# infil00p/openbts-ttsou

Hardware: AMD Instinct MI355X
Metric: Mbursts/s (156.25-sym @ 4 sps) demod+detect (higher is better)
Workload: dtype f32

## Files before the change

### openbts-ttsou_amd/csrc/trxsig_corr.h

```cpp
#pragma once
#include "trxsig_dev.h"

namespace {

template <int SPS>
struct CorrGeom {
  static constexpr int NL = 36 * SPS;
  static constexpr int NC = (NL + 15) / 16;
  static constexpr int FRONT = 8 * SPS;
  static constexpr int WPAD0 = NC * 16 + 15 * SPS + 1;
  static constexpr int WPAD = ((WPAD0 + 15) / 32) * 32 + 16;
  static constexpr int H = (5 * SPS + 1 > 12) ? 5 * SPS + 1 : 12;
  static constexpr int NS = 2 * H + 1;
  static constexpr int NE = 20 * SPS;
  static constexpr int NEQ = (NE + 15) / 16;
  static constexpr int NPAIR = (NS + 2) / 2;
};
template <typename T>
__device__ __forceinline__ T &rec_slot(T *rec, int Bpad, int s, int b) { return rec[2 * ((size_t)(s >> 1) * Bpad + b) + (s & 1)]; }

template <int N>
__device__ __forceinline__ float add_row_shl(float acc, float v) {
  float r;
  if (N == 0) asm volatile("v_add_f32 %0, %1, %2" : "=v"(r) : "v"(v), "v"(acc));
  else asm volatile("v_add_f32_dpp %0, %1, %2 row_shl:%3 row_mask:0xf bank_mask:0xf bound_ctrl:1"
                    : "=v"(r) : "v"(v), "v"(acc), "n"(N));
  return r;
}
template <int SPS, int I>
__device__ __forceinline__ float energy_chain_step(float acc, const float (&nrm)[CorrGeom<SPS>::NEQ]) {
  if constexpr (I < CorrGeom<SPS>::NE) {
    acc = add_row_shl<I % 16>(acc, nrm[I / 16]);
    return energy_chain_step<SPS, I + 1>(acc, nrm);
  } else {
    return acc;
  }
}
template <int SPS, int I>
__device__ __forceinline__ float energy_chain(float acc, const float (&nrm)[CorrGeom<SPS>::NEQ]) {
  asm volatile("s_nop 1");
  return energy_chain_step<SPS, I>(acc, nrm);
}

template <int SPS>
struct CorrIn {
  typedef CorrGeom<SPS> G;
  static constexpr int NW = (CorrGeom<SPS>::NL + 15) / 16;
  cx w[NW];
  cx e[CorrGeom<SPS>::NEQ];
  int b;
  bool live, good;
  __device__ __forceinline__ void stage_window(cx *W, int r) const {
#pragma unroll
    for (int i = 0; i < NW; i++) {
      const int q = r + 16 * i;
      if (q < G::NL) W[G::FRONT + q] = w[i];
    }
  }
  __device__ __forceinline__ void stage_norms(float *ef, int r) const {
#pragma unroll
    for (int q = 0; q < G::NEQ; q++) {
      const int i = r + 16 * q;
      if (i < G::NE) ef[i] = norm2(e[q]);
    }
  }
};

template <int SPS>
__device__ __forceinline__ void corr_issue(CorrIn<SPS> &in, int b, int B, int r, const cx *__restrict__ samples,
                                           const int32_t *__restrict__ offset, const int32_t *__restrict__ length) {
  typedef CorrGeom<SPS> G;
  in.b = b;
  in.live = b < B;
  int off = 0, len = 0;
  if (in.live) { off = offset[b]; len = length[b]; }
  in.good = in.live && (off >= 0) && (len >= 92 * SPS) && (len <= 157 * SPS) && (len % SPS == 0);
  const cx *x = samples + (in.good ? off : 0);
#pragma unroll
  for (int i = 0; i < CorrIn<SPS>::NW; i++) {
    const int q = r + 16 * i;
    in.w[i] = (in.good && q < G::NL) ? x[56 * SPS + q] : mk(0, 0);
  }
#pragma unroll
  for (int q = 0; q < G::NEQ; q++) {
    const int i = r + 16 * q;
    in.e[q] = (in.good && i < G::NE) ? x[i] : mk(0, 0);
  }
}

template <int SPS, bool REC, bool EFIRST = false, unsigned TAPCLS = TRX_TAPS_GENERIC, typename IN = CorrIn<SPS>>
__device__ __forceinline__ void corr_round(const IN &in, cx *W, float4 *E, int lane, int r, const cx (&tap)[16],
                                           cx *__restrict__ rec, int Bpad, int &M_out, float &energy_out) {
  typedef CorrGeom<SPS> G;
  auto stage_norms = [&] { in.stage_norms(reinterpret_cast<float *>(E), r); };
  auto sum_norms = [&] {
    float energy = 0.0f;
#pragma unroll
    for (int i4 = 0; i4 < (G::NE + 3) / 4; i4++) {
      const float4 e = E[i4];
      energy = energy + e.x;
      if (4 * i4 + 1 < G::NE) energy = energy + e.y;
      if (4 * i4 + 2 < G::NE) energy = energy + e.z;
      if (4 * i4 + 3 < G::NE) energy = energy + e.w;
    }
    return energy;
  };
  float energy = 0.0f;
  if (EFIRST) {
    stage_norms();
    wave_lds_fence();
    energy = sum_norms();
    asm volatile("" : "+v"(energy));
    wave_lds_fence();
  }
  for (int q = r; q < G::FRONT; q += 16) W[q] = mk(0, 0);
  for (int q = G::FRONT + G::NL + r; q < G::WPAD; q += 16) W[q] = mk(0, 0);
  in.stage_window(W, r);
  if (!EFIRST) stage_norms();
  wave_lds_fence();
  if (!EFIRST) energy = sum_norms();

  float bestP = 0.0f;
  int bestT = -1;
  cx cval[G::NC];
  constexpr int CG = (SPS == 4) ? TRX_CORR_CG : 1;
  constexpr int UPC = 16 / SPS;
  constexpr int NU = UPC * (CG - 1) + 16;
#pragma unroll
  for (int c0 = 0; c0 < G::NC; c0 += CG) {
    cx sv[NU];
#pragma unroll
    for (int u = 0; u < NU; u++) sv[u] = W[r + 16 * c0 + SPS * u];
#pragma unroll
    for (int cc = 0; cc < CG; cc++) {
      if (c0 + cc < G::NC) {
        cx acc = mk(0, 0);
#pragma unroll
        for (int k = 15; k >= 0; k--) acc = cadd(acc, cmul_tap(sv[UPC * cc + k], tap[k], (TAPCLS >> (2 * k)) & 3));
        cval[c0 + cc] = acc;
      }
    }
  }
  wave_lds_fence();
#pragma unroll
  for (int c = 0; c < G::NC; c++) {
    const int t = r + 16 * c;
    if (t < G::NL) {
      W[t] = cval[c];
      const float p = norm2(cval[c]);
      if (p > bestP) { bestP = p; bestT = t; }
    }
  }
#pragma unroll
  for (int m = 1; m < 16; m <<= 1) {
    const float oP = __shfl_xor(bestP, m, 64);
    const int oT = __shfl_xor(bestT, m, 64);
    const bool take = (oP > bestP) || (oP == bestP && oT >= 0 && (bestT < 0 || oT < bestT));
    if (take) { bestP = oP; bestT = oT; }
  }
  wave_lds_fence();

  M_out = bestT;
  energy_out = energy;
  if (REC && in.live) {
    const int M = bestT;
    auto slot = [&](int s) {
      cx v = mk(0, 0);
      if (s < G::NS) {
        const int lag = M - G::H + s;
        if (lag >= 0 && lag < G::NL) v = W[lag];
      } else if (s == G::NS) {
        v = mk(__int_as_float(in.good ? M : -2), energy);
      }
      return v;
    };
    for (int j = r; j < G::NPAIR; j += 16) {
      const cx a = slot(2 * j), c = slot(2 * j + 1);
      reinterpret_cast<float4 *>(rec)[(size_t)j * Bpad + in.b] = make_float4(a.r, a.i, c.r, c.i);
    }
  }
  wave_lds_fence();
  (void)lane;
}


inline unsigned tap_classes(const TrxTables *hT, int tsc) {
  unsigned m = 0;
  for (int k = 0; k < 16; k++) {
    const trx_c32 a = hT->mid_ctap[tsc][k];
    const unsigned c = (a.r == 1.0f || a.r == -1.0f) ? 1u : ((a.i == 1.0f || a.i == -1.0f) ? 2u : 0u);
    m |= c << (2 * k);
  }
  return m;
}

}
```

### openbts-ttsou_amd/csrc/trxsig_dev.h

```cpp
#pragma once
#include <hip/hip_runtime.h>
#include <hip/hip_fp16.h>
#include <stdint.h>

#include <type_traits>

#include "trxsig_tables.h"
#include "trxsig_launch.h"

#ifndef TRX_CORR_CG
#define TRX_CORR_CG 3
#endif
#ifndef TRX_CORR_WPS
#define TRX_CORR_WPS 1
#endif
#ifndef TRX_CORR_ROUNDS
#define TRX_CORR_ROUNDS 1
#endif
#ifndef TRX_DEMOD_WAVES
#define TRX_DEMOD_WAVES 4
#endif

namespace {

typedef trx_c32 cx;

__device__ __forceinline__ cx mk(float r, float i) { cx z; z.r = r; z.i = i; return z; }
__device__ __forceinline__ cx cmul(cx x, cx a) { return mk(x.r * a.r - x.i * a.i, x.r * a.i + x.i * a.r); }
__device__ __forceinline__ cx cmul_sum(cx x, cx a, float nai) { return mk(x.r * a.r + x.i * nai, x.r * a.i + x.i * a.r); }
__device__ __forceinline__ float neg_opaque(float v) {
  float r = -v;
  asm volatile("" : "+v"(r));
  return r;
}
__device__ __forceinline__ cx cmul_sum(cx x, cx a) { return cmul_sum(x, a, neg_opaque(a.i)); }
__device__ __forceinline__ cx cmulr(cx x, float a) { return mk(x.r * a, x.i * a); }
__device__ __forceinline__ cx cadd(cx x, cx a) { return mk(x.r + a.r, x.i + a.i); }
__device__ __forceinline__ float norm2(cx x) { return x.i * x.i + x.r * x.r; }
__device__ __forceinline__ cx cinv(cx x) { float n = norm2(x); return mk(x.r / n, -x.i / n); }
__device__ __forceinline__ cx cdiv(cx x, cx a) { return cmul(x, cinv(a)); }

template <int CTRL>
__device__ __forceinline__ float dpp_f(float v) {
  return __int_as_float(__builtin_amdgcn_update_dpp(0, __float_as_int(v), CTRL, 0xf, 0xf, true));
}
template <int CTRL>
__device__ __forceinline__ int dpp_i(int v) { return __builtin_amdgcn_update_dpp(0, v, CTRL, 0xf, 0xf, true); }
__device__ __forceinline__ float wave_sum_any_order(float v) {
  v += dpp_f<0xB1>(v);
  v += dpp_f<0x4E>(v);
  v += dpp_f<0x141>(v);
  v += dpp_f<0x140>(v);
  const float r0 = __int_as_float(__builtin_amdgcn_readlane(__float_as_int(v), 0));
  const float r1 = __int_as_float(__builtin_amdgcn_readlane(__float_as_int(v), 16));
  const float r2 = __int_as_float(__builtin_amdgcn_readlane(__float_as_int(v), 32));
  const float r3 = __int_as_float(__builtin_amdgcn_readlane(__float_as_int(v), 48));
  return ((r0 + r1) + r2) + r3;
}
__device__ __forceinline__ void argmax_take(float &P, int &T, float oP, int oT) {
  const bool take = (oP > P) || (oP == P && oT >= 0 && (T < 0 || oT < T));
  P = take ? oP : P;
  T = take ? oT : T;
}
__device__ __forceinline__ void wave_argmax(float &P, int &T) {
  argmax_take(P, T, dpp_f<0xB1>(P), dpp_i<0xB1>(T));
  argmax_take(P, T, dpp_f<0x4E>(P), dpp_i<0x4E>(T));
  argmax_take(P, T, dpp_f<0x141>(P), dpp_i<0x141>(T));
  argmax_take(P, T, dpp_f<0x140>(P), dpp_i<0x140>(T));
  float bp = __int_as_float(__builtin_amdgcn_readlane(__float_as_int(P), 0));
  int bt = __builtin_amdgcn_readlane(T, 0);
#pragma unroll
  for (int r = 16; r < 64; r += 16)
    argmax_take(bp, bt, __int_as_float(__builtin_amdgcn_readlane(__float_as_int(P), r)), __builtin_amdgcn_readlane(T, r));
  P = bp; T = bt;
}

typedef float v2f __attribute__((ext_vector_type(2)));
__device__ __forceinline__ v2f pk(cx z) { v2f v = {z.r, z.i}; return v; }
__device__ __forceinline__ v2f pk_cmul(v2f x, v2f a) {
  v2f p, q, r;
  asm("v_pk_mul_f32 %0, %1, %2 op_sel_hi:[0,1]" : "=v"(p) : "v"(x), "v"(a));
  asm("v_pk_mul_f32 %0, %1, %2 op_sel:[1,1] op_sel_hi:[1,0]" : "=v"(q) : "v"(x), "v"(a));
  asm("v_pk_add_f32 %0, %1, %2 neg_lo:[0,1]" : "=v"(r) : "v"(p), "v"(q));
  return r;
}
__device__ __forceinline__ v2f pk_mul(v2f x, v2f a) {
  v2f r;
  asm("v_pk_mul_f32 %0, %1, %2" : "=v"(r) : "v"(x), "v"(a));
  return r;
}
template <int HI>
__device__ __forceinline__ v2f pk_mul_tap(v2f x, v2f t) {
  v2f r;
  if (HI) asm("v_pk_mul_f32 %0, %1, %2 op_sel:[0,1] op_sel_hi:[1,1]" : "=v"(r) : "v"(x), "v"(t));
  else asm("v_pk_mul_f32 %0, %1, %2 op_sel_hi:[1,0]" : "=v"(r) : "v"(x), "v"(t));
  return r;
}
__device__ __forceinline__ v2f pk_csub(v2f x, v2f a) {
  v2f r;
  asm("v_pk_add_f32 %0, %1, %2 neg_lo:[0,1] neg_hi:[0,1]" : "=v"(r) : "v"(x), "v"(a));
  return r;
}
__device__ __forceinline__ cx unpk(v2f v) { return mk(v.x, v.y); }
__device__ __forceinline__ v2f pk_cadd(v2f x, v2f a) {
  v2f r;
  asm("v_pk_add_f32 %0, %1, %2" : "=v"(r) : "v"(x), "v"(a));
  return r;
}

struct SmpC32 {
  static constexpr int kBytes = 8;
  static __device__ __forceinline__ cx ld(const void *base, long long i) { return reinterpret_cast<const cx *>(base)[i]; }
  typedef cx raw_t;
  static __device__ __forceinline__ raw_t ldraw(const void *base, long long i) { return reinterpret_cast<const cx *>(base)[i]; }
  static __device__ __forceinline__ raw_t zero() { return mk(0, 0); }
  static __device__ __forceinline__ cx widen(raw_t r) { return r; }
  static __device__ __forceinline__ float4 ld2(const void *base, long long first, int q) {
    return reinterpret_cast<const float4 *>(reinterpret_cast<const cx *>(base) + first)[q];
  }
};
struct SmpF16 {
  static constexpr int kBytes = 4;
  static __device__ __forceinline__ cx ld(const void *base, long long i) {
    const float2 v = __half22float2(reinterpret_cast<const __half2 *>(base)[i]);
    return mk(v.x, v.y);
  }
  typedef unsigned raw_t;
  static __device__ __forceinline__ raw_t ldraw(const void *base, long long i) { return reinterpret_cast<const unsigned *>(base)[i]; }
  static __device__ __forceinline__ raw_t zero() { return 0u; }
  static __device__ __forceinline__ cx widen(raw_t r) {
    const float2 v = __half22float2(*reinterpret_cast<const __half2 *>(&r));
    return mk(v.x, v.y);
  }
  static __device__ __forceinline__ float4 ld2(const void *base, long long first, int q) {
    const uint2 u = reinterpret_cast<const uint2 *>(reinterpret_cast<const __half2 *>(base) + first)[q];
    const float2 a = __half22float2(*reinterpret_cast<const __half2 *>(&u.x)), b = __half22float2(*reinterpret_cast<const __half2 *>(&u.y));
    return make_float4(a.x, a.y, b.x, b.y);
  }
};

struct TapArg { float v[32]; };

#define TRX_TAPS_GENERIC 0u
template <int SPS> struct TapPattern {
  static constexpr unsigned value = (SPS == 4) ? 0x19999999u : 0x99999999u;
};
__device__ __forceinline__ float fma_steer(float a, float b, float c) {
  float r;
  asm("v_fma_f32 %0, %1, %2, %3 ; steering" : "=v"(r) : "v"(a), "v"(b), "v"(c));
  return r;
}
__device__ __forceinline__ float fma_steer_s(float a, float b_sgpr, float c) {
  float r;
  asm("v_fma_f32 %0, %1, %2, %3 ; steering" : "=v"(r) : "v"(a), "s"(b_sgpr), "v"(c));
  return r;
}
__device__ __forceinline__ cx cmul_tap(cx x, cx a, int cls) {
  if (cls == 1) {
    const float p = x.i * a.i, q = x.r * a.i;
    cx z;
    asm("v_fma_f32 %0, %2, %4, -%5 ; exact-product\n\tv_fma_f32 %1, %3, %4, %6 ; exact-product"
        : "=&v"(z.r), "=v"(z.i) : "v"(x.r), "v"(x.i), "s"(a.r), "v"(p), "v"(q));
    return z;
  }
  if (cls == 2) {
    const float p = x.r * a.r, q = x.i * a.r;
    cx z;
    asm("v_fma_f32 %0, %3, -%4, %5 ; exact-product\n\tv_fma_f32 %1, %2, %4, %6 ; exact-product"
        : "=&v"(z.r), "=v"(z.i) : "v"(x.r), "v"(x.i), "s"(a.i), "v"(p), "v"(q));
    return z;
  }
  return cmul(x, a);
}

#define TRX_PI_F 3.14159274101257324f
#define TRX_2PI_F 6.28318548202514648f

template <int N>
__device__ __forceinline__ float row_shl(float v) {
  if (N == 0) return v;
  return __int_as_float(__builtin_amdgcn_update_dpp(0, __float_as_int(v), 0x100 + N, 0xf, 0xf, true));
}

__device__ __forceinline__ void lds_barrier() {
  asm volatile("s_waitcnt lgkmcnt(0)\n\ts_barrier" ::: "memory");
}
__device__ __forceinline__ void wave_lds_fence() {
  __builtin_amdgcn_fence(__ATOMIC_RELEASE, "wavefront");
  __builtin_amdgcn_wave_barrier();
  __builtin_amdgcn_fence(__ATOMIC_ACQUIRE, "wavefront");
}

__device__ __forceinline__ float dev_range_reduce(float arg) {
  if (arg > 1.0F) arg = arg - (ceilf(arg) - 1.0F);
  if (arg < 0.0F) arg = arg + ceilf(-arg);
  return arg;
}
__device__ __forceinline__ float dev_sin_lookup(const float *__restrict__ sinT, float x) {
  const float arg = dev_range_reduce(x * (1 / TRX_2PI_F));
  const float argT = arg * (float)TRX_TABLESIZE;
  int argI = (int)argT;
  argI = argI < 0 ? 0 : (argI > TRX_TABLESIZE ? TRX_TABLESIZE : argI);
  const float delta = argT - argI;
  const float iDelta = 1.0F - delta;
  return iDelta * sinT[argI] + delta * sinT[argI + 1];
}
#define TRX_FSHIFT_MAXPHASE 25000.0f
__device__ __forceinline__ cx dev_expj_lookup(const TrxTables *__restrict__ T, float x) {
  const float arg = dev_range_reduce(x * (1 / TRX_2PI_F));
  const float argT = arg * (float)TRX_TABLESIZE;
  int argI = (int)argT;
  argI = argI < 0 ? 0 : (argI > TRX_TABLESIZE ? TRX_TABLESIZE : argI);
  const float delta = argT - argI;
  const float iDelta = 1.0F - delta;
  return mk(iDelta * T->cosT[argI] + delta * T->cosT[argI + 1], iDelta * T->sinT[argI] + delta * T->sinT[argI + 1]);
}
__device__ __forceinline__ float dev_sinc(const float *__restrict__ sinT, float x) {
  if ((x >= 0.01F) || (x <= -0.01F)) return dev_sin_lookup(sinT, x) / x;
  return 1.0F;
}

}
```

### openbts-ttsou_amd/csrc/trxsig_normal.hip

```cpp
#include "trxsig_bisect.h"
#include "trxsig_corr.h"
#include "trxsig_demod.h"
#include "trxsig_rxgen.h"

#ifndef TRX_RXC_WPS
#define TRX_RXC_WPS 1
#endif
#ifndef TRX_RXD_WPS
#define TRX_RXD_WPS 1
#endif

namespace {

template <int SPS, unsigned TAPCLS>
__global__ __launch_bounds__(256, TRX_CORR_WPS) void k_tsc_corr(const TrxTables *__restrict__ T,
                                                  const cx *__restrict__ samples,
                                                  const int32_t *__restrict__ offset,
                                                  const int32_t *__restrict__ length, int B, TapArg taps,
                                                  cx *__restrict__ rec, int Bpad) {
  typedef CorrGeom<SPS> G;
  static_assert(8 * G::WPAD >= 4 * G::NE, "the energy norms are staged in the row itself");
  __shared__ __attribute__((aligned(16))) cx rows[16][G::WPAD];
  (void)T;
  const int lane = threadIdx.x & 63, wave = threadIdx.x >> 6;
  const int row = lane >> 4, r = lane & 15;
  const int slot = wave * 4 + row;

  cx tap[16];
#pragma unroll
  for (int k = 0; k < 16; k++) tap[k] = mk(taps.v[2 * k], taps.v[2 * k + 1]);

  typedef CorrIn<SPS> In;
  In in[TRX_CORR_ROUNDS];
#pragma unroll
  for (int i = 0; i < TRX_CORR_ROUNDS; i++)
    corr_issue<SPS>(in[i], (blockIdx.x * TRX_CORR_ROUNDS + i) * 16 + slot, B, r, samples, offset, length);
#pragma unroll
  for (int i = 0; i < TRX_CORR_ROUNDS; i++) {
    int M;
    float energy;
    corr_round<SPS, true, true, TAPCLS, In>(in[i], rows[slot], reinterpret_cast<float4 *>(rows[slot]), lane, r, tap, rec, Bpad, M, energy);
  }
}


#ifdef TRX_TUNING_BUILD
template <int SPS>
__global__ __launch_bounds__(64) void k_tsc_peak(const TrxTables *__restrict__ T,
                                                 const cx *__restrict__ rec, int Bpad, int B, int tsc,
                                                 float detect_thresh, float energy_thresh,
                                                 uint8_t *__restrict__ flags, cx *__restrict__ amp_out,
                                                 float *__restrict__ toa_out,
                                                 float *__restrict__ avgpwr_out) {
  typedef CorrGeom<SPS> G;
  __shared__ cx loc[26][64];
  __shared__ float pw[G::NS][64];
  const int lane = threadIdx.x;
  const int b = blockIdx.x * 64 + lane;
  const bool live = b < B;
  const int bb = live ? b : B - 1;

  const cx meta = rec_slot(rec, Bpad, G::NS, bb);
  const int M = __float_as_int(meta.r);
  const float energy = meta.i;
  const bool good = M != -2;
#pragma unroll
  for (int s = 0; s < G::NS; s++) {
    const cx v = rec_slot(rec, Bpad, s, bb);
    pw[s][lane] = norm2(v);
    const int j = s - (G::H - 12);
    if (j >= 0 && j < 24) {
      const int lag = M - 12 + j;
      loc[j][lane] = (lag > G::NL - 2) ? mk(0, 0) : v;
    }
  }
  loc[24][lane] = mk(0, 0);
  loc[25][lane] = mk(0, 0);

  float peakIx;
  const cx peak = peak_bisect<64>(T->sinc_grid, loc, lane, M, &peakIx);

  float toa = peakIx;
  cx amp = peak;
  bool detected = false;
  const bool energy_ok = good && (energy_thresh < 0.0f ||
                                  energy / (float)(unsigned)G::NE > energy_thresh * energy_thresh);
  if (!(toa < 0.0f) && !(toa > (float)G::NL) && good) {
    const int p = (int)rintf(toa);
    float valley = 0.0f;
    int numRms = 0;
#pragma unroll
    for (int i = 2 * SPS; i <= 5 * SPS; i++) {
      const int lo = p - i, hi = p + i;
      int slo = lo - M + G::H, shi = hi - M + G::H;
      slo = slo < 0 ? 0 : slo; shi = shi > G::NS - 1 ? G::NS - 1 : shi;
      const float vlo = pw[slo][lane], vhi = pw[shi][lane];
      if (lo >= 0) { valley += vlo; numRms++; }
      if (hi < G::NL) { valley += vhi; numRms++; }
    }
    if (numRms < 2) {
      amp = mk(0, 0);
    } else {
      const float RMS = (float)((double)sqrtf(valley / (float)numRms) + 0.00001);
      const float peakToMean = sqrtf(norm2(amp)) / RMS;
      amp = cdiv(amp, T->mid_gain[tsc]);
      toa = toa - T->mid_toa[tsc];
      toa = toa - (float)((66 - 56) * SPS);
      detected = peakToMean > detect_thresh;
    }
  } else {
    amp = mk(0, 0);
  }
  if (!energy_ok) { amp = mk(0, 0); toa = 0.0f; detected = false; }

  if (live) {
    uint8_t fl = 0;
    if (!good) fl = TRXSIG_F_BADLEN;
    else fl = (energy_ok ? TRXSIG_F_ENERGY : 0) | (detected ? TRXSIG_F_DETECT : 0);
    flags[b] = fl;
    amp_out[b] = amp;
    toa_out[b] = toa;
    if (avgpwr_out) avgpwr_out[b] = good ? energy / (float)(unsigned)G::NE : 0.0f;
  }
}


template <int SPS>
struct Peak8Geom {
  typedef CorrGeom<SPS> G;
  static constexpr int NV = 2 * (3 * SPS + 1);
  static constexpr int O_PW = 26 * 2;
  static constexpr int O_V = O_PW + ((G::NS + 3) & ~3);
  static constexpr int STRIDE = O_V + ((NV + 3) & ~3);
};

template <int SPS>
__global__ __launch_bounds__(256, 8) void k_tsc_peak8(const TrxTables *__restrict__ T, const cx *__restrict__ rec, int Bpad,
                                                   int B, cx gain_inv, float mid_toa, float detect_thresh,
                                                   float energy_thresh, uint8_t *__restrict__ flags,
                                                   cx *__restrict__ amp_out, float *__restrict__ toa_out,
                                                   float *__restrict__ avgpwr_out) {
  typedef CorrGeom<SPS> G;
  typedef Peak8Geom<SPS> P8;
  __shared__ __attribute__((aligned(16))) float stab[32][24];
  __shared__ __attribute__((aligned(16))) float scratch[32][P8::STRIDE];
  {
    float tv[3];
#pragma unroll
    for (int k = 0; k < 3; k++) { const int ix = threadIdx.x * 3 + k; tv[k] = T->sinc_grid[16 * (ix / 24)][ix % 24]; }
#pragma unroll
    for (int k = 0; k < 3; k++) { const int ix = threadIdx.x * 3 + k; stab[ix / 24][ix % 24] = tv[k]; }
  }
  const int lane = threadIdx.x & 63;
  const int r = lane & 7;
  const int slot = threadIdx.x >> 3;
  const int b = blockIdx.x * 32 + slot;
  const bool live = b < B;
  const int bb = live ? b : B - 1;
  float *S = scratch[slot];
  cx *loc = reinterpret_cast<cx *>(S);
  float *pw = S + P8::O_PW, *V = S + P8::O_V;

  const cx meta = rec_slot(rec, Bpad, G::NS, bb);
  const int M = __float_as_int(meta.r);
  const float energy = meta.i;
  const bool good = M != -2;
#pragma unroll
  for (int s0 = 0; s0 < G::NS; s0 += 8) {
    const int sl = s0 + r;
    if (sl < G::NS) {
      const cx v = rec_slot(rec, Bpad, sl, bb);
      pw[sl] = norm2(v);
      const int j = sl - (G::H - 12);
      if (j >= 0 && j < 24) loc[j] = (M - 12 + j > G::NL - 2) ? mk(0, 0) : v;
    }
  }
  if (r < 2) loc[24 + r] = mk(0, 0);
  __syncthreads();

  int e = 0;
  asm volatile("" : "+v"(e));
  bool active = true;
  cx peak = mk(0, 0);
  {
    const int rel2 = kFusedRel2.v[r], rel1 = kFusedRel1.v[r];
#pragma unroll
    for (int st = 0; st < 4; st++) {
      const int inc_last = 128 >> (2 * st);
      const int el = e + (rel2 >> 2) * inc_last;
      float srow[24];
      if (st < 3) {
        const float4 *rw = reinterpret_cast<const float4 *>(stab[(el & 511) >> 4]);
#pragma unroll
        for (int q = 0; q < 6; q++) {
          const float4 t4 = rw[q];
          srow[4 * q] = t4.x; srow[4 * q + 1] = t4.y; srow[4 * q + 2] = t4.z; srow[4 * q + 3] = t4.w;
        }
      } else {
        fused_row(T, el, srow);
      }
      const cx pt = fused_point(loc, el, rel2 & 3, srow);
      fused_decide<8, 2, false>(pt, lane, 2 * inc_last, e, active, peak);
    }
    {
      float srow[24];
      fused_row(T, e, srow);
      const cx pt = fused_point(loc, e, rel1 & 3, srow);
      fused_decide<8, 1, false>(pt, lane, 1, e, active, peak);
    }
    float srow[24];
    fused_row(T, e, srow);
    peak = fused_point(loc, e, 1, srow);
    asm volatile("" : "+v"(peak.r), "+v"(peak.i));
  }
  cx amp;
  float toa;
  bool detected, energy_ok;
  fused_tail<SPS, 8>([&](int lag) { const int sl = lag - M + G::H; return (sl < 0 || sl >= G::NS) ? 0.0f : pw[sl]; }, V, r, M, e,
                     peak, good, energy, gain_inv, mid_toa, detect_thresh, energy_thresh, amp, toa, detected, energy_ok);
  if (live && r == 0) {
    uint8_t fl = 0;
    if (!good) fl = TRXSIG_F_BADLEN;
    else fl = (energy_ok ? TRXSIG_F_ENERGY : 0) | (detected ? TRXSIG_F_DETECT : 0);
    flags[b] = fl;
    amp_out[b] = amp;
    toa_out[b] = toa;
    if (avgpwr_out) avgpwr_out[b] = good ? energy / (float)(unsigned)G::NE : 0.0f;
  }
}



#endif

#ifndef TRX_PEAK2_THREADS
#define TRX_PEAK2_THREADS 512
#endif
constexpr int kPeak2Threads = TRX_PEAK2_THREADS;
template <int SPS>
__global__ __launch_bounds__(kPeak2Threads) void k_tsc_peak2(const TrxTables *__restrict__ T, const cx *__restrict__ rec, int Bpad,
                                                   int B, cx gain_inv, float mid_toa, float detect_thresh,
                                                   float energy_thresh, uint8_t *__restrict__ flags,
                                                   cx *__restrict__ amp_out, float *__restrict__ toa_out,
                                                   float *__restrict__ avgpwr_out) {
  typedef CorrGeom<SPS> G;
  constexpr int NL = G::NL, NE = G::NE, NP = 3 * SPS + 3;
  __shared__ __attribute__((aligned(16))) SincLds stab;
  const int tid = threadIdx.x;
  const int h = tid & 1;
  const int b = blockIdx.x * (kPeak2Threads / 2) + (tid >> 1);
  const bool live = b < B;
  const int bb = live ? b : B - 1;
#ifdef TRX_PEAK_PROBE
  long long pt_[16] = {0};
  int pk_ = 0;
#define TRX_STAMP() pt_[pk_++] = clock64()
#else
#define TRX_STAMP()
#endif
  TRX_STAMP();

  float4 tv[3072 / kPeak2Threads];
  sinc_lds_issue<kPeak2Threads>(T, tid, tv);
  const cx meta = rec_slot(rec, Bpad, G::NS, bb);
  const int M = __float_as_int(meta.r);
  const float energy = meta.i;
  const bool good = M != -2;
  const float4 *rec4 = reinterpret_cast<const float4 *>(rec);
  cx q[23];
  {
    constexpr int S0 = G::H - 12, P0 = S0 >> 1;
    float4 pw[12];
#pragma unroll
    for (int i = 0; i < 12; i++) pw[i] = rec4[(size_t)(P0 + h + i) * Bpad + bb];
#pragma unroll
    for (int k = 0; k < 23; k++) {
      const int ix = k + 2 * h;
      const float4 p4 = pw[((S0 + k) >> 1) - P0];
      const cx v = ((S0 + k) & 1) ? mk(p4.z, p4.w) : mk(p4.x, p4.y);
      q[k] = (M - 12 + ix > NL - 2) ? mk(0, 0) : v;
    }
  }
  cx vmine_[NP];
  constexpr int VLO = G::H - (5 * SPS + 1), VHI = G::H + (2 * SPS - 1);
  if constexpr ((VLO & 1) == 0 && (VHI & 1) == 0) {
    float4 pv[(NP + 1) / 2];
#pragma unroll
    for (int i = 0; i < (NP + 1) / 2; i++) pv[i] = rec4[(size_t)(((h ? VHI : VLO) >> 1) + i) * Bpad + bb];
#pragma unroll
    for (int k = 0; k < NP; k++) vmine_[k] = (k & 1) ? mk(pv[k >> 1].z, pv[k >> 1].w) : mk(pv[k >> 1].x, pv[k >> 1].y);
  } else {
#pragma unroll
    for (int k = 0; k < NP; k++) vmine_[k] = rec_slot(rec, Bpad, (h ? VHI : VLO) + k, bb);
  }
  sinc_lds_store<kPeak2Threads>(stab, tid, tv);
  TRX_STAMP();
  __syncthreads();
  TRX_STAMP();

  int e;
  const cx peak = pair_bisect(stab, q, h, e);
  TRX_STAMP();
  const float early = (float)(M - 1) + (float)e * 0.001953125f;
  float toa = early + 1.0f;
  cx amp = peak;
  bool detected = false;
  const bool energy_ok = good && (energy_thresh < 0.0f || energy / (float)(unsigned)NE > energy_thresh * energy_thresh);
  const bool sane = !(toa < 0.0f) && !(toa > (float)NL) && good;
  if (sane) {
    const int pk = (int)rintf(toa);
    const int a = pk - M + 1;
    float plo[NP], phi[NP];
#pragma unroll
    for (int k = 0; k < NP; k++) {
      const float mine = norm2(vmine_[k]);
      const float other = __int_as_float(__builtin_amdgcn_update_dpp(0, __float_as_int(mine), 0xB1, 0xf, 0xf, true));
      plo[k] = h ? other : mine; phi[k] = h ? mine : other;
    }
    float valley = 0.0f;
#pragma unroll
    for (int i = 2 * SPS; i <= 5 * SPS; i++) {
      const int t = 5 * SPS - i, u = i - 2 * SPS;
      const float vlo = a == 0 ? plo[t] : (a == 1 ? plo[t + 1] : plo[t + 2]);
      const float vhi = a == 0 ? phi[u] : (a == 1 ? phi[u + 1] : phi[u + 2]);
      valley = valley + vlo;
      valley = valley + vhi;
    }
    int nlo = (pk < 5 * SPS ? pk : 5 * SPS) - 2 * SPS + 1;
    int nhi = (NL - 1 - pk < 5 * SPS ? NL - 1 - pk : 5 * SPS) - 2 * SPS + 1;
    nlo = nlo < 0 ? 0 : nlo; nhi = nhi < 0 ? 0 : nhi;
    const int numRms = nlo + nhi;
    if (numRms < 2) {
      amp = mk(0, 0);
    } else {
      const float RMS = (float)((double)sqrtf(valley / (float)numRms) + 0.00001);
      const float peakToMean = sqrtf(norm2(amp)) / RMS;
      amp = cmul(amp, gain_inv);
      toa = toa - mid_toa;
      toa = toa - (float)((66 - 56) * SPS);
      detected = peakToMean > detect_thresh;
    }
  } else {
    amp = mk(0, 0);
  }
  if (!energy_ok) { amp = mk(0, 0); toa = 0.0f; detected = false; }

  if (live && h == 0) {
    uint8_t fl = 0;
    if (!good) fl = TRXSIG_F_BADLEN;
    else fl = (energy_ok ? TRXSIG_F_ENERGY : 0) | (detected ? TRXSIG_F_DETECT : 0);
    flags[b] = fl;
    amp_out[b] = amp;
    toa_out[b] = toa;
    if (avgpwr_out) avgpwr_out[b] = good ? energy / (float)(unsigned)G::NE : 0.0f;
  }
#ifdef TRX_PEAK_PROBE
  TRX_STAMP();
  if (live && avgpwr_out) {
    long long v = 0;
    for (int k = 1; k < 16; k++) if ((b & 15) == k) v = pt_[k] - pt_[0];
    if (h == 0) avgpwr_out[b] = (float)v;
  }
#endif
#undef TRX_STAMP
}

template <int SPS, unsigned TAPCLS>
__global__ __launch_bounds__(256, TRX_RXC_WPS) void k_tsc_corr_rx(TrxRxGen a, int B, TapArg taps, cx *__restrict__ rec, int Bpad) {
  static_assert(SPS == 4, "the fused front end is the 260 : 96 resampler");
  typedef CorrGeom<SPS> G;
  constexpr int XCAP = 160;
  static_assert(G::WPAD >= XCAP, "the raw stretch is parked in the burst's own row");
  __shared__ __attribute__((aligned(16))) cx rows[16][G::WPAD];
  __shared__ float4 tpb_s[RXG_NT];
  if (threadIdx.x < RXG_NT) tpb_s[threadIdx.x] = a.tpb[threadIdx.x];
  __syncthreads();
  const int lane = threadIdx.x & 63, wave = threadIdx.x >> 6;
  const int row = lane >> 4, r = lane & 15;
  const int slot = wave * 4 + row;
  cx tap[16];
#pragma unroll
  for (int k = 0; k < 16; k++) tap[k] = mk(taps.v[2 * k], taps.v[2 * k + 1]);
  const int b = blockIdx.x * 16 + slot;
  CorrIn<SPS> in;
  in.b = b; in.live = b < B; in.good = in.live;
  const RxBurst u = rx_burst(a, in.live ? b : 0);
  const int jlo = rx_index(u.g0, a.skipD).j0 - 3;
  cx *X = rows[slot];
  {
    short2 v[XCAP / 16];
#pragma unroll
    for (int i = 0; i < XCAP / 16; i++) v[i] = rx_raw(a, u.s, jlo + r + 16 * i);
#pragma unroll
    for (int i = 0; i < XCAP / 16; i++) X[r + 16 * i] = rx_widen(a, v[i]);
  }
  wave_lds_fence();
  {
    static_assert(G::NL % 16 == 0 && G::NE % 16 == 0, "every lane owns a sample in every round");
    const int nb = rx_boundary(u.g0);
    RxIdx ix = rx_index(u.g0 + 56 * SPS + r, a.skipD);
#pragma unroll
    for (int i = 0; i < CorrIn<SPS>::NW; i++) {
      in.w[i] = rx_sample(X, tpb_s, jlo, ix, nb - (56 * SPS + r + 16 * i), a.w0, a.w1);
      ix = rx_step<16>(ix);
      if (i % 3 == 2) asm volatile("" : "+v"(in.w[i].r), "+v"(in.w[i].i), "+v"(in.w[i - 1].r), "+v"(in.w[i - 1].i), "+v"(in.w[i - 2].r), "+v"(in.w[i - 2].i) : : "memory");
    }
    ix = rx_index(u.g0 + r, a.skipD);
#pragma unroll
    for (int q = 0; q < G::NEQ; q++) {
      in.e[q] = rx_sample(X, tpb_s, jlo, ix, nb - (r + 16 * q), a.w0, a.w1);
      ix = rx_step<16>(ix);
      if (q % 3 == 2) asm volatile("" : "+v"(in.e[q].r), "+v"(in.e[q].i), "+v"(in.e[q - 1].r), "+v"(in.e[q - 1].i), "+v"(in.e[q - 2].r), "+v"(in.e[q - 2].i) : : "memory");
    }
  }
  wave_lds_fence();
  int M;
  float energy;
  corr_round<SPS, true, true, TAPCLS>(in, rows[slot], reinterpret_cast<float4 *>(rows[slot]), lane, r, tap, rec, Bpad, M, energy);
}

template <int SPS, bool TOL = false>
__global__ __launch_bounds__(64 * TRX_DEMOD_WAVES, TRX_RXD_WPS) void k_demod_rx(const TrxTables *__restrict__ T, TrxRxGen a, int B,
                                                                  const cx *__restrict__ amp_in, const float *__restrict__ toa_in,
                                                                  const uint8_t *__restrict__ flags, int need_mask,
                                                                  float *__restrict__ soft, uint8_t *__restrict__ hard, int nsoft,
                                                                  int stride) {
  static_assert(SPS == 4, "the fused front end is the 260 : 96 resampler");
  typedef DemodGeom<SPS, 148> G;
  constexpr int XCAP = 256;
  static_assert(G::U >= XCAP, "the raw stretch is parked in the burst's staging area");
  __shared__ cx ph[TRX_DEMOD_WAVES][G::U];
  __shared__ float4 tpb_s[RXG_NT];
  if (threadIdx.x < RXG_NT) tpb_s[threadIdx.x] = a.tpb[threadIdx.x];
  __syncthreads();
  const int lane = threadIdx.x & 63;
  const int wave = __builtin_amdgcn_readfirstlane(threadIdx.x >> 6);
  const int b = blockIdx.x * TRX_DEMOD_WAVES + wave;
  if (b >= B) return;
  float *sb = soft + (size_t)b * stride;
  uint8_t *hb = hard ? hard + (size_t)b * stride : nullptr;
  const cx amp = amp_in[b];
  const float toa = toa_in[b];
  bool enabled = fabsf(toa) <= 4096.0f;
  if (flags) enabled = enabled && (need_mask ? ((flags[b] & need_mask) == need_mask) : (flags[b] != 0));
  if (!enabled) {
    for (int m = lane; m < nsoft; m += 64) { sb[m] = 0.0f; if (hb) hb[m] = 0; }
    return;
  }
  const RxBurst u = rx_burst(a, b);
  const int jlo = rx_index(u.g0, a.skipD).j0 - 3;
  cx *X = ph[wave];
  {
    short2 v[XCAP / 64];
#pragma unroll
    for (int i = 0; i < XCAP / 64; i++) v[i] = rx_raw(a, u.s, jlo + lane + 64 * i);
#pragma unroll
    for (int i = 0; i < XCAP / 64; i++) X[lane + 64 * i] = rx_widen(a, v[i]);
  }
  wave_lds_fence();
  constexpr int NSL = (157 * SPS + 63) / 64;
  cx sv[NSL];
  {
    const int nb = rx_boundary(u.g0);
    RxIdx ix = rx_index(u.g0 + lane, a.skipD);
#pragma unroll
    for (int i = 0; i < NSL; i++) {
      sv[i] = rx_sample(X, tpb_s, jlo, ix, nb - (lane + 64 * i), a.w0, a.w1);
      ix = rx_step<64>(ix);
      if (i % 2 == 1) asm volatile("" : "+v"(sv[i].r), "+v"(sv[i].i), "+v"(sv[i - 1].r), "+v"(sv[i - 1].i) : : "memory");
    }
  }
  const int N = u.N;
  auto stage = [&](cx *P, cx inv, int lo) {
    typedef DemodGeom<SPS, 148> D;
    const int u0 = lane + lo;
    if (u0 >= 0) {
      cx *p0 = P + (u0 % SPS) * D::QLEN + u0 / SPS;
#pragma unroll
      for (int i = 0; i < NSL; i++)
        if (lane + 64 * i < N && u0 + 64 * i < D::U) p0[i * (64 / SPS)] = cmul(sv[i], inv);
    } else {
#pragma unroll
      for (int i = 0; i < NSL; i++) {
        const int uu = u0 + 64 * i;
        if (lane + 64 * i < N && uu >= 0 && uu < D::U) P[(uu % SPS) * D::QLEN + uu / SPS] = cmul(sv[i], inv);
      }
    }
  };
  if (TOL) {
    float xm = 0.0f;
#pragma unroll
    for (int i = 0; i < NSL; i++)
      if (lane + 64 * i < N) xm = max3_abs(sv[i].r, sv[i].i, xm);
    auto stage_raw = [&](cx *P, int lo) {
      typedef DemodGeom<SPS, 148> D;
      const int u0 = lane + lo;
      if (u0 >= 0) {
        cx *p0 = P + (u0 % SPS) * D::QLEN + u0 / SPS;
#pragma unroll
        for (int i = 0; i < NSL; i++)
          if (lane + 64 * i < N && u0 + 64 * i < D::U) p0[i * (64 / SPS)] = sv[i];
      } else {
#pragma unroll
        for (int i = 0; i < NSL; i++) {
          const int uu = u0 + 64 * i;
          if (lane + 64 * i < N && uu >= 0 && uu < D::U) P[(uu % SPS) * D::QLEN + uu / SPS] = sv[i];
        }
      }
    };
    if (fused_demod_tol_ex<SPS>(T, ph[wave], N, amp, toa, lane, sb, hb, nsoft, xm, stage_raw)) return;
  }
  fused_demod_ex<SPS, 64>(T, ph[wave], N, amp, toa, lane, sb, hb, nsoft, stage, [] {}, nullptr, nullptr);
}

}

int trx_rec_slots(int sps) {
  switch (sps) {
    case 1: return 2 * CorrGeom<1>::NPAIR;
    case 2: return 2 * CorrGeom<2>::NPAIR;
    case 4: return 2 * CorrGeom<4>::NPAIR;
  }
  return 0;
}

template <int S>
static void launch_tsc_detect(hipStream_t st, const TrxTables *dT, const TrxTables *hT, const trx_c32 *samples, const int32_t *off,
                              const int32_t *len, int B, int tsc, float detect_thresh, float energy_thresh,
                              trx_c32 *rec, int Bpad, uint8_t *flags, trx_c32 *amp, float *toa, float *avgpwr,
                              int variant, TrxProfiler *prof) {
  TapArg ta;
  for (int k = 0; k < 16; k++) { ta.v[2 * k] = hT->mid_ctap[tsc][k].r; ta.v[2 * k + 1] = hT->mid_ctap[tsc][k].i; }
  if (prof) prof->begin(TRXSIG_K_TSC_CORR, st);
  const dim3 cgrid((B + 16 * TRX_CORR_ROUNDS - 1) / (16 * TRX_CORR_ROUNDS));
  if (!(variant & 1) && tap_classes(hT, tsc) == TapPattern<S>::value)
    k_tsc_corr<S, TapPattern<S>::value><<<cgrid, dim3(256), 0, st>>>(dT, samples, off, len, B, ta, rec, Bpad);
  else
    k_tsc_corr<S, TRX_TAPS_GENERIC><<<cgrid, dim3(256), 0, st>>>(dT, samples, off, len, B, ta, rec, Bpad);
  if (prof) { prof->end(TRXSIG_K_TSC_CORR, st); prof->begin(TRXSIG_K_TSC_PEAK, st); }
  const trx_c32 g = hT->mid_gain[tsc];
  const float n = g.i * g.i + g.r * g.r;
  trx_c32 ginv; ginv.r = g.r / n; ginv.i = -g.i / n;
#ifdef TRX_TUNING_BUILD
  if (variant & 4) {
    k_tsc_peak<S><<<dim3((B + 63) / 64), dim3(64), 0, st>>>(dT, rec, Bpad, B, tsc, detect_thresh, energy_thresh,
                                                            flags, amp, toa, avgpwr);
  } else if (variant & 2) {
    k_tsc_peak8<S><<<dim3((B + 31) / 32), dim3(256), 0, st>>>(dT, rec, Bpad, B, ginv, hT->mid_toa[tsc], detect_thresh,
                                                              energy_thresh, flags, amp, toa, avgpwr);
  } else
#endif
  {
    k_tsc_peak2<S><<<dim3((B + kPeak2Threads / 2 - 1) / (kPeak2Threads / 2)), dim3(kPeak2Threads), 0, st>>>(dT, rec, Bpad, B, ginv, hT->mid_toa[tsc], detect_thresh,
                                                                energy_thresh, flags, amp, toa, avgpwr);
  }
  if (prof) prof->end(TRXSIG_K_TSC_PEAK, st);
}

namespace {
__global__ __launch_bounds__(256) void k_copy_verdict(const uint8_t *__restrict__ f, const cx *__restrict__ a, const float *__restrict__ t, int B,
                                                      uint8_t *__restrict__ fo, cx *__restrict__ ao, float *__restrict__ to) {
  const int b = blockIdx.x * 256 + threadIdx.x;
  if (b >= B) return;
  fo[b] = f[b]; ao[b] = a[b]; to[b] = t[b];
}
}
hipError_t trx_launch_copy_verdict(hipStream_t st, const uint8_t *flags, const trx_c32 *amp, const float *toa, int B, uint8_t *flags_out,
                                   trx_c32 *amp_out, float *toa_out) {
  if (B <= 0) return hipSuccess;
  k_copy_verdict<<<dim3((B + 255) / 256), dim3(256), 0, st>>>(flags, amp, toa, B, flags_out, amp_out, toa_out);
  return hipGetLastError();
}

hipError_t trx_launch_tsc_detect(hipStream_t st, int sps, const TrxTables *dT, const TrxTables *hT, const trx_c32 *samples,
                                 const int32_t *off, const int32_t *len, int B, int tsc,
                                 float detect_thresh, float energy_thresh, trx_c32 *rec, int Bpad,
                                 uint8_t *flags, trx_c32 *amp, float *toa, float *avgpwr, int variant,
                                 TrxProfiler *prof) {
  if (B <= 0) return hipSuccess;
  switch (sps) {
    case 1: launch_tsc_detect<1>(st, dT, hT, samples, off, len, B, tsc, detect_thresh, energy_thresh, rec, Bpad, flags, amp, toa, avgpwr, variant, prof); break;
    case 2: launch_tsc_detect<2>(st, dT, hT, samples, off, len, B, tsc, detect_thresh, energy_thresh, rec, Bpad, flags, amp, toa, avgpwr, variant, prof); break;
    case 4: launch_tsc_detect<4>(st, dT, hT, samples, off, len, B, tsc, detect_thresh, energy_thresh, rec, Bpad, flags, amp, toa, avgpwr, variant, prof); break;
    default: return hipErrorInvalidValue;
  }
  return hipGetLastError();
}

hipError_t trx_launch_rx_normal(hipStream_t st, const TrxTables *dT, const TrxTables *hT, const TrxRxGen &gen, int B, int tsc,
                                float detect_thresh, float energy_thresh, trx_c32 *rec, int Bpad, uint8_t *flags, trx_c32 *amp,
                                float *toa, float *avgpwr, float *soft, uint8_t *hard, int nsoft, int stride, int generic_taps,
                                TrxProfiler *prof, int soft_tolerance) {
  if (B <= 0) return hipSuccess;
  if (nsoft > 148 || gen.nb <= 0) return hipErrorInvalidValue;
  constexpr int S = 4;
  TapArg ta;
  for (int k = 0; k < 16; k++) { ta.v[2 * k] = hT->mid_ctap[tsc][k].r; ta.v[2 * k + 1] = hT->mid_ctap[tsc][k].i; }
  if (prof) prof->begin(TRXSIG_K_TSC_CORR, st);
  const dim3 cgrid((B + 15) / 16);
  if (!generic_taps && tap_classes(hT, tsc) == TapPattern<S>::value)
    k_tsc_corr_rx<S, TapPattern<S>::value><<<cgrid, dim3(256), 0, st>>>(gen, B, ta, rec, Bpad);
  else
    k_tsc_corr_rx<S, TRX_TAPS_GENERIC><<<cgrid, dim3(256), 0, st>>>(gen, B, ta, rec, Bpad);
  if (prof) { prof->end(TRXSIG_K_TSC_CORR, st); prof->begin(TRXSIG_K_TSC_PEAK, st); }
  const trx_c32 g = hT->mid_gain[tsc];
  const float n = g.i * g.i + g.r * g.r;
  trx_c32 ginv; ginv.r = g.r / n; ginv.i = -g.i / n;
  k_tsc_peak2<S><<<dim3((B + kPeak2Threads / 2 - 1) / (kPeak2Threads / 2)), dim3(kPeak2Threads), 0, st>>>(dT, rec, Bpad, B, ginv, hT->mid_toa[tsc], detect_thresh, energy_thresh,
                                                              flags, amp, toa, avgpwr);
  if (prof) prof->end(TRXSIG_K_TSC_PEAK, st);
  if (nsoft > 0) {
    if (prof) prof->begin(TRXSIG_K_DEMOD, st);
    if (soft_tolerance)
      k_demod_rx<S, true><<<dim3((B + TRX_DEMOD_WAVES - 1) / TRX_DEMOD_WAVES), dim3(64 * TRX_DEMOD_WAVES), 0, st>>>(
          dT, gen, B, amp, toa, flags, TRXSIG_F_DETECT, soft, hard, nsoft, stride);
    else
      k_demod_rx<S><<<dim3((B + TRX_DEMOD_WAVES - 1) / TRX_DEMOD_WAVES), dim3(64 * TRX_DEMOD_WAVES), 0, st>>>(
          dT, gen, B, amp, toa, flags, TRXSIG_F_DETECT, soft, hard, nsoft, stride);
    if (prof) prof->end(TRXSIG_K_DEMOD, st);
  }
  return hipGetLastError();
}

hipError_t trx_launch_rx_demod(hipStream_t st, const TrxTables *dT, const TrxRxGen &gen, int B, const trx_c32 *amp, const float *toa,
                               const uint8_t *flags, int need_mask, float *soft, uint8_t *hard, int nsoft, int stride, TrxProfiler *prof,
                               int soft_tolerance) {
  if (B <= 0 || nsoft <= 0) return hipSuccess;
  if (nsoft > 148 || gen.nb <= 0) return hipErrorInvalidValue;
  if (prof) prof->begin(TRXSIG_K_DEMOD, st);
  if (soft_tolerance)
    k_demod_rx<4, true><<<dim3((B + TRX_DEMOD_WAVES - 1) / TRX_DEMOD_WAVES), dim3(64 * TRX_DEMOD_WAVES), 0, st>>>(dT, gen, B, amp, toa, flags,
                                                                                                                  need_mask, soft, hard, nsoft, stride);
  else
    k_demod_rx<4><<<dim3((B + TRX_DEMOD_WAVES - 1) / TRX_DEMOD_WAVES), dim3(64 * TRX_DEMOD_WAVES), 0, st>>>(dT, gen, B, amp, toa, flags, need_mask,
                                                                                                            soft, hard, nsoft, stride);
  if (prof) prof->end(TRXSIG_K_DEMOD, st);
  return hipGetLastError();
}

hipError_t trx_launch_demod(hipStream_t st, int sps, const TrxTables *dT, const trx_c32 *samples,
                            const int32_t *off, const int32_t *len, int B, const trx_c32 *amp,
                            const float *toa, const uint8_t *flags, int need_mask, float *soft,
                            uint8_t *hard, int nsoft, int stride, TrxProfiler *prof, int soft_tolerance) {
  if (B <= 0) return hipSuccess;
  const dim3 grid((B + TRX_DEMOD_WAVES - 1) / TRX_DEMOD_WAVES), block(64 * TRX_DEMOD_WAVES);
  if (prof) prof->begin(TRXSIG_K_DEMOD, st);
#define TRX_DEMOD_CASE(S)                                                                                          \
  case S:                                                                                                          \
    if (nsoft <= 148 && soft_tolerance)                                                                            \
      k_demod<S, false, 148, SmpC32, true><<<grid, block, 0, st>>>(dT, samples, off, len, B, amp, toa, flags, need_mask, soft, hard, \
                                                     nsoft, stride);                                              \
    else if (nsoft <= 148)                                                                                         \
      k_demod<S, false, 148><<<grid, block, 0, st>>>(dT, samples, off, len, B, amp, toa, flags, need_mask, soft, hard, \
                                                     nsoft, stride);                                              \
    else                                                                                                           \
      k_demod<S, false, 157><<<grid, block, 0, st>>>(dT, samples, off, len, B, amp, toa, flags, need_mask, soft, hard, \
                                                     nsoft, stride);                                              \
    break;
  switch (sps) {
    TRX_DEMOD_CASE(1)
    TRX_DEMOD_CASE(2)
    TRX_DEMOD_CASE(4)
    default: return hipErrorInvalidValue;
  }
#undef TRX_DEMOD_CASE
  if (prof) prof->end(TRXSIG_K_DEMOD, st);
  return hipGetLastError();
}
```

Measured before the change: 629.5.

## Specialize correlator for near-unit taps with runtime magnitude screen and pad skipping

Correlation kernels are now templated on a 64-bit tap spec that records which taps are exactly ±1 or ±j (tiny imaginary part) and their signs. For those taps the complex multiply becomes a plain add or subtract. Tap products that only touch zero padding are skipped at compile time. A wave-wide screen on the window's exponent range (finite values, bounded dynamic range) decides at runtime whether the trimmed path is numerically safe. Otherwise the full path runs, with a NaN/Inf poison fix-up so the output still matches generic semantics. This adds code size, five kernel instantiations, and extra DPP reductions per round.

```diff
diff --git a/openbts-ttsou_amd/csrc/trxsig_corr.h b/openbts-ttsou_amd/csrc/trxsig_corr.h
--- a/openbts-ttsou_amd/csrc/trxsig_corr.h
+++ b/openbts-ttsou_amd/csrc/trxsig_corr.h
@@ -1,4 +1,6 @@
 #pragma once
+#include <cmath>
+
 #include "trxsig_dev.h"
 
 namespace {
@@ -57,6 +59,22 @@
       if (q < G::NL) W[G::FRONT + q] = w[i];
     }
   }
+  __device__ __forceinline__ void window_extremes(unsigned &lo, unsigned &hi) const {
+    static_assert(G::NL % 16 == 0, "every lane holds NW samples of the window");
+    lo = 0xffffffffu; hi = 0u;
+#pragma unroll
+    for (int i = 0; i < NW; i++) {
+      const unsigned a = __float_as_uint(w[i].r) & 0x7fffffffu, c = __float_as_uint(w[i].i) & 0x7fffffffu;
+      lo = min(lo, min(a, c));
+      hi = max(hi, max(a, c));
+    }
+  }
+  __device__ __forceinline__ unsigned window_max() const {
+    unsigned hi = 0u;
+#pragma unroll
+    for (int i = 0; i < NW; i++) hi = max(hi, max(__float_as_uint(w[i].r) & 0x7fffffffu, __float_as_uint(w[i].i) & 0x7fffffffu));
+    return hi;
+  }
   __device__ __forceinline__ void stage_norms(float *ef, int r) const {
 #pragma unroll
     for (int q = 0; q < G::NEQ; q++) {
@@ -88,7 +106,81 @@
   }
 }
 
-template <int SPS, bool REC, bool EFIRST = false, unsigned TAPCLS = TRX_TAPS_GENERIC, typename IN = CorrIn<SPS>>
+template <int SPS>
+constexpr bool corr_pad_only(int c, int k) {
+  const int first = 16 * c + SPS * k, last = first + 15;
+  return last < CorrGeom<SPS>::FRONT || first >= CorrGeom<SPS>::FRONT + CorrGeom<SPS>::NL;
+}
+
+template <int SPS>
+__device__ __forceinline__ bool corr_screen(const CorrIn<SPS> &in, unsigned &hi) {
+  unsigned lo;
+  in.window_extremes(lo, hi);
+  lo = min(lo, (unsigned)dpp_i<0xB1>((int)lo));  hi = max(hi, (unsigned)dpp_i<0xB1>((int)hi));
+  lo = min(lo, (unsigned)dpp_i<0x4E>((int)lo));  hi = max(hi, (unsigned)dpp_i<0x4E>((int)hi));
+  lo = min(lo, (unsigned)dpp_i<0x141>((int)lo)); hi = max(hi, (unsigned)dpp_i<0x141>((int)hi));
+  lo = min(lo, (unsigned)dpp_i<0x140>((int)lo)); hi = max(hi, (unsigned)dpp_i<0x140>((int)hi));
+  const bool ok = hi < 0x7f800000u && lo >= (27u << 23) && lo + (20u << 23) >= hi;
+  return __builtin_amdgcn_ballot_w64(!ok) == 0;
+}
+
+template <int SPS>
+__device__ __forceinline__ unsigned corr_row_max(const CorrIn<SPS> &in) {
+  unsigned hi = in.window_max();
+  hi = max(hi, (unsigned)dpp_i<0xB1>((int)hi));
+  hi = max(hi, (unsigned)dpp_i<0x4E>((int)hi));
+  hi = max(hi, (unsigned)dpp_i<0x141>((int)hi));
+  return max(hi, (unsigned)dpp_i<0x140>((int)hi));
+}
+
+template <int SPS>
+__device__ __forceinline__ void corr_poison(unsigned hi, const cx *W, int r, cx (&cval)[CorrGeom<SPS>::NC]) {
+  if constexpr (SPS > 1) {
+    if (hi >= 0x7f800000u) {
+#pragma unroll
+      for (int c = 0; c < CorrGeom<SPS>::NC; c++) {
+        unsigned worst = 0u;
+#pragma unroll 1
+        for (int m = 1; m < 16 * SPS; m++) {
+          if (m % SPS == 0) continue;
+          const cx x = W[r + 16 * c + m];
+          worst = max(worst, max(__float_as_uint(x.r) & 0x7fffffffu, __float_as_uint(x.i) & 0x7fffffffu));
+        }
+        if (worst >= 0x7f800000u) cval[c] = mk(__uint_as_float(0x7fc00000u), __uint_as_float(0x7fc00000u));
+      }
+    }
+  }
+}
+
+template <int SPS, tapspec_t TAPS, bool TRIM>
+__device__ __forceinline__ void corr_sums(const cx *W, int r, const cx (&tap)[16], cx (&cval)[CorrGeom<SPS>::NC]) {
+  typedef CorrGeom<SPS> G;
+  constexpr bool SPEC = TAPS != TRX_TAPS_GENERIC;
+  constexpr int CG = (SPS == 4) ? TRX_CORR_CG : 1;
+  constexpr int UPC = 16 / SPS;
+  constexpr int NU = UPC * (CG - 1) + 16;
+#pragma unroll
+  for (int c0 = 0; c0 < G::NC; c0 += CG) {
+    cx sv[NU];
+#pragma unroll
+    for (int u = 0; u < NU; u++) sv[u] = W[r + 16 * c0 + SPS * u];
+#pragma unroll
+    for (int cc = 0; cc < CG; cc++) {
+      if (c0 + cc < G::NC) {
+        cx acc = mk(0, 0);
+#pragma unroll
+        for (int k = 15; k >= 0; k--) {
+          if (SPEC && corr_pad_only<SPS>(c0 + cc, k)) continue;
+          if (TRIM && ((tap_tiny_mask(TAPS) >> k) & 1)) acc = cacc_tiny(acc, sv[UPC * cc + k], tap_cls(TAPS, k), (tap_neg_mask(TAPS) >> k) & 1);
+          else acc = cadd(acc, cmul_tap(sv[UPC * cc + k], tap[k], tap_cls(TAPS, k)));
+        }
+        cval[c0 + cc] = acc;
+      }
+    }
+  }
+}
+
+template <int SPS, bool REC, bool EFIRST = false, tapspec_t TAPS = TRX_TAPS_GENERIC, typename IN = CorrIn<SPS>>
 __device__ __forceinline__ void corr_round(const IN &in, cx *W, float4 *E, int lane, int r, const cx (&tap)[16],
                                            cx *__restrict__ rec, int Bpad, int &M_out, float &energy_out) {
   typedef CorrGeom<SPS> G;
@@ -116,6 +208,11 @@
   for (int q = r; q < G::FRONT; q += 16) W[q] = mk(0, 0);
   for (int q = G::FRONT + G::NL + r; q < G::WPAD; q += 16) W[q] = mk(0, 0);
   in.stage_window(W, r);
+  constexpr bool TINY = tap_tiny_mask(TAPS) != 0;
+  bool trim = false;
+  unsigned hi = 0u;
+  if constexpr (TINY) trim = corr_screen<SPS>(in, hi);
+  else if constexpr (SPS > 1) hi = corr_row_max<SPS>(in);
   if (!EFIRST) stage_norms();
   wave_lds_fence();
   if (!EFIRST) energy = sum_norms();
@@ -123,22 +220,18 @@
   float bestP = 0.0f;
   int bestT = -1;
   cx cval[G::NC];
-  constexpr int CG = (SPS == 4) ? TRX_CORR_CG : 1;
-  constexpr int UPC = 16 / SPS;
-  constexpr int NU = UPC * (CG - 1) + 16;
-#pragma unroll
-  for (int c0 = 0; c0 < G::NC; c0 += CG) {
-    cx sv[NU];
-#pragma unroll
-    for (int u = 0; u < NU; u++) sv[u] = W[r + 16 * c0 + SPS * u];
-#pragma unroll
-    for (int cc = 0; cc < CG; cc++) {
-      if (c0 + cc < G::NC) {
-        cx acc = mk(0, 0);
-#pragma unroll
-        for (int k = 15; k >= 0; k--) acc = cadd(acc, cmul_tap(sv[UPC * cc + k], tap[k], (TAPCLS >> (2 * k)) & 3));
-        cval[c0 + cc] = acc;
-      }
+  if constexpr (!TINY) {
+    corr_sums<SPS, TAPS, false>(W, r, tap, cval);
+    corr_poison<SPS>(hi, W, r, cval);
+  } else {
+    int rb = r;
+    if (trim) {
+      asm volatile("" : "+v"(rb));
+      corr_sums<SPS, TAPS, true>(W, rb, tap, cval);
+    } else {
+      asm volatile("" : "+v"(rb));
+      corr_sums<SPS, TAPS, false>(W, rb, tap, cval);
+      corr_poison<SPS>(hi, W, r, cval);
     }
   }
   wave_lds_fence();
@@ -188,10 +281,47 @@
   unsigned m = 0;
   for (int k = 0; k < 16; k++) {
     const trx_c32 a = hT->mid_ctap[tsc][k];
+    if (!std::isfinite(a.r) || !std::isfinite(a.i)) return TRX_TAPS_GENERIC;
     const unsigned c = (a.r == 1.0f || a.r == -1.0f) ? 1u : ((a.i == 1.0f || a.i == -1.0f) ? 2u : 0u);
     m |= c << (2 * k);
   }
   return m;
 }
-
-}
+inline tapspec_t tap_spec(const TrxTables *hT, int tsc) {
+  const unsigned cls = tap_classes(hT, tsc);
+  unsigned tiny = 0, neg = 0;
+  for (int k = 0; k < 16; k++) {
+    const trx_c32 a = hT->mid_ctap[tsc][k];
+    const int c = (cls >> (2 * k)) & 3;
+    if (c == 0) continue;
+    const float unit = (c == 1) ? a.r : a.i, other = (c == 1) ? a.i : a.r;
+    if (std::fabs(other) <= 0x1p-50f) { tiny |= 1u << k; if (unit < 0.0f) neg |= 1u << k; }
+  }
+  return tap_spec_of(cls, tiny, neg);
+}
+constexpr bool tap_spec_fits(tapspec_t have, tapspec_t built) {
+  return (unsigned)have == (unsigned)built && (tap_tiny_mask(built) & ~tap_tiny_mask(have)) == 0 &&
+         (tap_neg_mask(have) & tap_tiny_mask(built)) == tap_neg_mask(built);
+}
+template <int SPS> struct TapSpecs {
+  static constexpr int N = 1;
+  static constexpr tapspec_t at(int) { return tap_spec_of(TapPattern<SPS>::value, 0, 0); }
+};
+template <> struct TapSpecs<4> {
+  static constexpr int N = 5;
+  static constexpr tapspec_t at(int i) {
+    constexpr unsigned neg[N] = {0x000Bu, 0x0008u, 0x0009u, 0x0809u, 0x0801u};
+    return tap_spec_of(TapPattern<4>::value, TapPattern<4>::tiny, neg[i]);
+  }
+};
+template <int SPS, int I = 0, typename F>
+inline void launch_for_taps(const TrxTables *hT, int tsc, bool generic_taps, F &&launch) {
+  if constexpr (I < TapSpecs<SPS>::N) {
+    if (!generic_taps && tap_spec_fits(tap_spec(hT, tsc), TapSpecs<SPS>::at(I))) launch(std::integral_constant<tapspec_t, TapSpecs<SPS>::at(I)>{});
+    else launch_for_taps<SPS, I + 1>(hT, tsc, generic_taps, launch);
+  } else {
+    launch(std::integral_constant<tapspec_t, (tapspec_t)TRX_TAPS_GENERIC>{});
+  }
+}
+
+}
diff --git a/openbts-ttsou_amd/csrc/trxsig_dev.h b/openbts-ttsou_amd/csrc/trxsig_dev.h
--- a/openbts-ttsou_amd/csrc/trxsig_dev.h
+++ b/openbts-ttsou_amd/csrc/trxsig_dev.h
@@ -144,6 +144,7 @@
 #define TRX_TAPS_GENERIC 0u
 template <int SPS> struct TapPattern {
   static constexpr unsigned value = (SPS == 4) ? 0x19999999u : 0x99999999u;
+  static constexpr unsigned tiny = (SPS == 4) ? 0x080Bu : 0u;
 };
 __device__ __forceinline__ float fma_steer(float a, float b, float c) {
   float r;
@@ -171,6 +172,18 @@
     return z;
   }
   return cmul(x, a);
+}
+
+typedef unsigned long long tapspec_t;
+constexpr tapspec_t tap_spec_of(unsigned cls, unsigned tiny, unsigned neg) {
+  return (tapspec_t)cls | ((tapspec_t)(tiny & 0xffffu) << 32) | ((tapspec_t)(neg & tiny & 0xffffu) << 48);
+}
+constexpr int tap_cls(tapspec_t t, int k) { return (int)(t >> (2 * k)) & 3; }
+constexpr unsigned tap_tiny_mask(tapspec_t t) { return (unsigned)(t >> 32) & 0xffffu; }
+constexpr unsigned tap_neg_mask(tapspec_t t) { return (unsigned)(t >> 48) & 0xffffu; }
+__device__ __forceinline__ cx cacc_tiny(cx acc, cx x, int cls, bool neg) {
+  if (cls == 1) return neg ? mk(acc.r - x.r, acc.i - x.i) : mk(acc.r + x.r, acc.i + x.i);
+  return neg ? mk(acc.r + x.i, acc.i - x.r) : mk(acc.r - x.i, acc.i + x.r);
 }
 
 #define TRX_PI_F 3.14159274101257324f
diff --git a/openbts-ttsou_amd/csrc/trxsig_normal.hip b/openbts-ttsou_amd/csrc/trxsig_normal.hip
--- a/openbts-ttsou_amd/csrc/trxsig_normal.hip
+++ b/openbts-ttsou_amd/csrc/trxsig_normal.hip
@@ -12,7 +12,7 @@
 
 namespace {
 
-template <int SPS, unsigned TAPCLS>
+template <int SPS, tapspec_t TAPCLS>
 __global__ __launch_bounds__(256, TRX_CORR_WPS) void k_tsc_corr(const TrxTables *__restrict__ T,
                                                   const cx *__restrict__ samples,
                                                   const int32_t *__restrict__ offset,
@@ -365,7 +365,7 @@
 #undef TRX_STAMP
 }
 
-template <int SPS, unsigned TAPCLS>
+template <int SPS, tapspec_t TAPCLS>
 __global__ __launch_bounds__(256, TRX_RXC_WPS) void k_tsc_corr_rx(TrxRxGen a, int B, TapArg taps, cx *__restrict__ rec, int Bpad) {
   static_assert(SPS == 4, "the fused front end is the 260 : 96 resampler");
   typedef CorrGeom<SPS> G;
@@ -533,10 +533,9 @@
   for (int k = 0; k < 16; k++) { ta.v[2 * k] = hT->mid_ctap[tsc][k].r; ta.v[2 * k + 1] = hT->mid_ctap[tsc][k].i; }
   if (prof) prof->begin(TRXSIG_K_TSC_CORR, st);
   const dim3 cgrid((B + 16 * TRX_CORR_ROUNDS - 1) / (16 * TRX_CORR_ROUNDS));
-  if (!(variant & 1) && tap_classes(hT, tsc) == TapPattern<S>::value)
-    k_tsc_corr<S, TapPattern<S>::value><<<cgrid, dim3(256), 0, st>>>(dT, samples, off, len, B, ta, rec, Bpad);
-  else
-    k_tsc_corr<S, TRX_TAPS_GENERIC><<<cgrid, dim3(256), 0, st>>>(dT, samples, off, len, B, ta, rec, Bpad);
+  launch_for_taps<S>(hT, tsc, variant & 1, [&](auto spec) {
+    k_tsc_corr<S, decltype(spec)::value><<<cgrid, dim3(256), 0, st>>>(dT, samples, off, len, B, ta, rec, Bpad);
+  });
   if (prof) { prof->end(TRXSIG_K_TSC_CORR, st); prof->begin(TRXSIG_K_TSC_PEAK, st); }
   const trx_c32 g = hT->mid_gain[tsc];
   const float n = g.i * g.i + g.r * g.r;
@@ -598,10 +597,9 @@
   for (int k = 0; k < 16; k++) { ta.v[2 * k] = hT->mid_ctap[tsc][k].r; ta.v[2 * k + 1] = hT->mid_ctap[tsc][k].i; }
   if (prof) prof->begin(TRXSIG_K_TSC_CORR, st);
   const dim3 cgrid((B + 15) / 16);
-  if (!generic_taps && tap_classes(hT, tsc) == TapPattern<S>::value)
-    k_tsc_corr_rx<S, TapPattern<S>::value><<<cgrid, dim3(256), 0, st>>>(gen, B, ta, rec, Bpad);
-  else
-    k_tsc_corr_rx<S, TRX_TAPS_GENERIC><<<cgrid, dim3(256), 0, st>>>(gen, B, ta, rec, Bpad);
+  launch_for_taps<S>(hT, tsc, generic_taps != 0, [&](auto spec) {
+    k_tsc_corr_rx<S, decltype(spec)::value><<<cgrid, dim3(256), 0, st>>>(gen, B, ta, rec, Bpad);
+  });
   if (prof) { prof->end(TRXSIG_K_TSC_CORR, st); prof->begin(TRXSIG_K_TSC_PEAK, st); }
   const trx_c32 g = hT->mid_gain[tsc];
   const float n = g.i * g.i + g.r * g.r;
```

After: 645.9 (median of 6 runs). No clear change (+2.6%).
